# xuyuan/waymo_2d_tracking

Measured on AMD Instinct MI355X. Metric: end-to-end frames/sec (detect+SORT) on 1920x1280 Waymo frames, higher is better.
Workload: dtype f32; 1 GPU; Cascade R-CNN X152-32x8d-FPN dconv (random-init, fp32, batch 1) on synthetic 1920x1280x3 frames -> top-100 detections/frame -> SORT (max_age 2, min_hits 0, all boxes tracked; trackers resident for the whole segment); 5 cameras x 2 frames per step per GPU; 1x1 and dense 3x3 convolutions: f32 operands as exact 3 x bf16 splits, six cross terms on the bf16 matrix cores, f32 accumulate (csrc/det_gemm_s; stage=e2e, parallelism=sequence-shard x1

## Files before the change

### include/waymodet.h

```cpp
#ifndef WAYMODET_H
#define WAYMODET_H
#include <stddef.h>
#include <stdint.h>
#ifdef __cplusplus
extern "C" {
#endif

int wd_roi_pool_fpn_f32(const float* const* feats, const int32_t* heights, const int32_t* widths,
                        const float* scales, int n_levels, int channels, int batch,
                        const float* rois, int n_rois, int pooled, int min_level, int canonical_level,
                        float canonical_size, float* out, void* stream);

size_t wd_nms_workspace(int n);
int wd_select_kept(const uint8_t* keep_mask, const uint8_t* valid, const int64_t* order, int n, int cap, int64_t* out_idx,
                   int32_t* count, void* stream);
int wd_nms_sorted_f32(const float* boxes, const int32_t* idxs, int n, float iou_threshold,
                      uint8_t* keep_mask, int32_t* n_keep, void* workspace, size_t workspace_bytes, void* stream);

size_t wd_gemm_nt_workspace(int M, int N, int K);
int wd_gemm_nt_ws_f32(const float* A, const float* Bt, const float* bias, const float* residual, int relu, int M, int N, int K,
                      float* C, void* workspace, size_t workspace_bytes, void* stream);

int wd_gemm_lt_f32(const float* a, const float* w, const float* bias, const float* residual, float* out, int m, int n, int k,
                   int relu, void* workspace, size_t workspace_bytes, void* stream);
int wd_gemm_lt_plan_info(int m, int n, int k, int relu, int has_bias, int has_residual, float* best_us, int* candidates);
size_t wd_gemm_split_packed_bytes(int N, int K);
int wd_gemm_split_pack_weight(const float* w, int N, int K, void* packed, void* stream);
int wd_gemm_split_pack_weight_strided(const float* w, int N, int K, long stride_n, long stride_k, void* packed, void* stream);
typedef struct WdSplitPackDesc {
    const float* src;
    void* dst;
    long s_n, s_c, s_kh, s_kw;
    long first_block;
    int N, K, C, ksize, flip, reserved;
} WdSplitPackDesc;
int wd_gemm_split_pack_batch(const WdSplitPackDesc* descs_device, int count, long total_blocks, void* stream);
size_t wd_gemm_split_workspace(long M, int N, int K);
int wd_gemm_split_f32(const float* a, long lda, const void* packed_w, const float* bias, const float* residual, float* out, long ldc,
                      int M, int N, int K, int relu, void* workspace, size_t workspace_bytes, void* stream);
int wd_conv_split_f32(const float* x, int batch, int H, int W, int C, const void* packed_w, int ksize, int stride, int pad, const float* bias,
                      const float* residual, float* out, int N, int relu, void* workspace, size_t workspace_bytes, void* stream);
int wd_gemm_split_supported(const float* a, long lda, const float* bias, const float* residual, const float* out, long ldc, long M, int N, int K);
int wd_conv_split_position_major(int batch, int H, int W, int ksize, int stride, int pad);
typedef struct WdSplitIO {
    const float* a;
    long lda;
    const void* a_planes;
    const float* residual;
    const void* residual_planes;
    float* out;
    void* out_planes;
    long ldc;
} WdSplitIO;
size_t wd_split_planes_bytes(long M, int K);
int wd_split_planes_pack_f32(const float* a, long lda, long M, int K, void* planes, void* stream);
int wd_split_planes_unpack_f32(const void* planes, long M, int K, float* out, long ldo, void* stream);
int wd_gemm_split_io(const WdSplitIO* io, const void* packed_w, const float* bias, int M, int N, int K, int relu, void* workspace,
                     size_t workspace_bytes, void* stream);
int wd_nms_segmented_f32(const float* boxes, const int32_t* idxs, const int32_t* seg_offsets, int n_seg, float iou_threshold,
                         uint8_t* keep_mask, int32_t* n_keep, void* workspace, size_t workspace_bytes, void* stream);

size_t wd_rpn_topk_workspace(const int* n_per_level, int n_levels, int k);
int wd_rpn_topk_decode_f32(const float* const* logits, const float* const* deltas, const float* const* anchors,
                           const int* n_per_level, int n_levels, int k, float img_h, float img_w, float scale_clamp,
                           float* out_boxes, float* out_scores, int32_t* out_group, uint8_t* out_valid, void* workspace,
                           size_t workspace_bytes, void* stream);
int wd_sort_candidates_f32(const float* boxes, const float* scores, const int32_t* group, const uint8_t* valid,
                           const uint8_t* valid2 , int n, float* out_boxes, float* out_scores, int32_t* out_group, uint8_t* out_valid, int64_t* out_order,
                           void* stream);
int wd_box_candidates_f32(const float* boxes, const float* s0, const float* s1, const float* s2, const int32_t* n_valid, int rows,
                          int num_classes, float score_thresh, float img_h, float img_w, float* out_boxes, float* out_scores,
                          int32_t* out_group, uint8_t* out_valid, int64_t* out_order, void* stream);
int wd_gather_kept_f32(const uint8_t* keep, const uint8_t* valid, const float* boxes, const float* scores, const int64_t* order,
                       int n, int cap, int num_classes, float* out_boxes, float* out_scores, int64_t* out_class, int32_t* count,
                       void* stream);
int wd_detections_to_wire(const float* boxes, const float* scores, const int64_t* classes, const int32_t* count, int n, int in_w,
                          int in_h, int hflip, int out_w, int out_h, double* xywhs, int32_t* category, void* stream);

size_t wd_deform_packed_weight_floats(int c_in, int c_out, int groups);
int wd_deform_pack_weight(const float* weight_oihw, int c_in, int c_out, int groups, float* packed, void* stream);
const char* wd_deform_conv3x3_variant(int c_in, int groups, int stride, int pad, int has_offset);
const char* wd_deform_conv3x3_last_kernel(void);
int wd_deform_conv3x3_f32(const float* x, const float* offset, const float* mask, const float* packed_weight,
                          const float* scale, const float* bias, int relu,
                          int batch, int h, int w, int c_in, int c_out, int groups, int stride, int pad,
                          float* y, void* stream);
int wd_deform_conv3x3_hint_f32(const float* x, const float* offset, const float* mask, const float* packed_weight,
                               const float* scale, const float* bias, int relu, int batch, int h, int w, int c_in,
                               int c_out, int groups, int stride, int pad, int far_offsets, float* y, void* stream);
size_t wd_deform_table_bytes(int batch, int h, int w);
int wd_deform_offsets_table_f32(const float* partial, int ld, const float* bias, int batch, int h, int w, float* offsets,
                                void* table, void* stream);
int wd_deform_conv3x3_tab_f32(const float* x, const float* offset, const float* mask, const float* packed_weight,
                              const float* scale, const float* bias, int relu, int batch, int h, int w, int c_in,
                              int c_out, int groups, int stride, int pad, int far_offsets, const void* table, float* y,
                              void* stream);
// ... 57 lines not shown
```

### waymo_2d_tracking_amd/csrc/det_gemm_split.hip

```cpp
#include "common.h"
#include "../../include/waymodet.h"
#include <cstdlib>
#include <cstring>

namespace {

using bf16x8 = __attribute__((ext_vector_type(8))) __bf16;
using bf16x2 = __attribute__((ext_vector_type(2))) __bf16;
using f32x2 = __attribute__((ext_vector_type(2))) float;
using f32x16 = __attribute__((ext_vector_type(16))) float;
using u32x4 = __attribute__((ext_vector_type(4))) unsigned;

constexpr int BK = 64;
constexpr int BN = 256;
constexpr int NTHREADS = 512;
constexpr int CHUNK = 6144;

struct SplitArgs {
    const float* a;
    const unsigned char* ap;
    const uint4* w;
    const float* bias;
    const float* residual;
    const unsigned char* resp;
    float* out;
    unsigned char* outp;
    long lda, ldc;
    int M, N, K, relu;
    int tiles_m, tiles_n;
    int splitk;
    float* part;
    long long* stamps;
    int H, W, C, Ho, Wo, stride, pad, ksize;
};

__device__ __forceinline__ unsigned pk_bf16(float a, float b) {
    const f32x2 v = {a, b};
    return __builtin_bit_cast(unsigned, __builtin_convertvector(v, bf16x2));
}

__device__ __forceinline__ void split_pair(float x0, float x1, unsigned& h, unsigned& m, unsigned& l) {
    h = pk_bf16(x0, x1);
    const float r0 = x0 - __uint_as_float(h << 16), r1 = x1 - __uint_as_float(h & 0xffff0000u);
    m = pk_bf16(r0, r1);
    const float s0 = r0 - __uint_as_float(m << 16), s1 = r1 - __uint_as_float(m & 0xffff0000u);
    l = pk_bf16(s0, s1);
}

__device__ __forceinline__ float bf_lo(unsigned v) { return __uint_as_float(v << 16); }
__device__ __forceinline__ float bf_hi(unsigned v) { return __uint_as_float(v & 0xffff0000u); }

__device__ __forceinline__ size_t planes_offset(int row, int col, int ncols) {
    return ((size_t)(row >> 5) * (size_t)(ncols >> 5) + (size_t)(col >> 5)) * CHUNK +
           (size_t)((row & 31) * 64 + ((((col >> 3) & 3) ^ ((row >> 2) & 3)) << 4) + ((col >> 2) & 1) * 8);
}

constexpr int LDC = BN + 8;

template <int MT>
__device__ __forceinline__ void split_epilogue(const SplitArgs& p, unsigned char* smem, const f32x16 (&acc)[MT], int m0, int n0, int wave, int lane, int mlim,
                                               int row_mul = 1, int row_add = 0) {
    const int rr = lane & 31, rg = lane >> 5;
    float* ct = reinterpret_cast<float*>(smem);
    const int ncols = p.N - n0 < BN ? p.N - n0 : BN;
    constexpr int PASS = 3;
    auto stage = [&](int i0) {
        if (i0 > 0) __builtin_amdgcn_s_barrier();
#pragma unroll
        for (int i = i0; i < i0 + PASS && i < MT; ++i)
#pragma unroll
            for (int e = 0; e < 16; ++e)
                ct[((i - i0) * 32 + (e & 3) + 8 * (e >> 2) + 4 * rg) * LDC + 32 * wave + rr] = acc[i][e];
        __builtin_amdgcn_s_waitcnt(0xC07F);
        __builtin_amdgcn_s_barrier();
    };
    if (p.outp == nullptr) {
        const int c4 = 4 * lane;
        float4 bv = make_float4(0.f, 0.f, 0.f, 0.f);
        if (p.bias && c4 < ncols) bv = *reinterpret_cast<const float4*>(p.bias + n0 + c4);
        constexpr int RPW = 32 * PASS / 8;
#pragma unroll
        for (int i0 = 0; i0 < MT; i0 += PASS) {
            const int nrows = 32 * ((MT - i0) < PASS ? (MT - i0) : PASS);
            float4 rv[RPW];
            if (p.residual) {
// ... 64 lines not shown
        stage(i0);
#pragma unroll
        for (int j = 0; j < UPW; ++j) {
            const int u = wave + 8 * j;
            if (u < nunits && m0 + 32 * (i0 + u / (2 * ncb)) < mlim) {
                const int rbi = u / (2 * ncb), cb = (u >> 1) - rbi * ncb, h = u & 1;
                const int r = 16 * h + ur, row = m0 + 32 * (i0 + rbi) + r;
                const int c8 = 8 * ((lane & 3) ^ ((r >> 2) & 3)), col = n0 + 32 * cb + c8;
                const float* src = ct + (32 * rbi + r) * LDC + 32 * cb + c8;
                float4 v0 = *reinterpret_cast<const float4*>(src), v1 = *reinterpret_cast<const float4*>(src + 4);
                if (p.bias) {
                    const float4 b0 = *reinterpret_cast<const float4*>(p.bias + col), b1 = *reinterpret_cast<const float4*>(p.bias + col + 4);
                    v0.x += b0.x; v0.y += b0.y; v0.z += b0.z; v0.w += b0.w; v1.x += b1.x; v1.y += b1.y; v1.z += b1.z; v1.w += b1.w;
                }
                if (p.resp) {
                    const uint4 hh = rq[j][0], mm = rq[j][1], ll = rq[j][2];
                    v0.x += (bf_lo(hh.x) + bf_lo(mm.x)) + bf_lo(ll.x); v0.y += (bf_hi(hh.x) + bf_hi(mm.x)) + bf_hi(ll.x);
                    v0.z += (bf_lo(hh.y) + bf_lo(mm.y)) + bf_lo(ll.y); v0.w += (bf_hi(hh.y) + bf_hi(mm.y)) + bf_hi(ll.y);
                    v1.x += (bf_lo(hh.z) + bf_lo(mm.z)) + bf_lo(ll.z); v1.y += (bf_hi(hh.z) + bf_hi(mm.z)) + bf_hi(ll.z);
                    v1.z += (bf_lo(hh.w) + bf_lo(mm.w)) + bf_lo(ll.w); v1.w += (bf_hi(hh.w) + bf_hi(mm.w)) + bf_hi(ll.w);
                } else if (p.residual) {
                    const uint4 q0 = rq[j][0], q1 = rq[j][1];
                    v0.x += __uint_as_float(q0.x); v0.y += __uint_as_float(q0.y); v0.z += __uint_as_float(q0.z); v0.w += __uint_as_float(q0.w);
                    v1.x += __uint_as_float(q1.x); v1.y += __uint_as_float(q1.y); v1.z += __uint_as_float(q1.z); v1.w += __uint_as_float(q1.w);
                }
                if (p.relu) {
                    v0.x = fmaxf(v0.x, 0.f); v0.y = fmaxf(v0.y, 0.f); v0.z = fmaxf(v0.z, 0.f); v0.w = fmaxf(v0.w, 0.f);
                    v1.x = fmaxf(v1.x, 0.f); v1.y = fmaxf(v1.y, 0.f); v1.z = fmaxf(v1.z, 0.f); v1.w = fmaxf(v1.w, 0.f);
                }
                if (p.out && row < mlim) {
                    float4* d = reinterpret_cast<float4*>(p.out + (size_t)row * p.ldc + col);
                    d[0] = v0; d[1] = v1;
                }
                unsigned hv[4], mv[4], lv[4];
                split_pair(v0.x, v0.y, hv[0], mv[0], lv[0]); split_pair(v0.z, v0.w, hv[1], mv[1], lv[1]);
                split_pair(v1.x, v1.y, hv[2], mv[2], lv[2]); split_pair(v1.z, v1.w, hv[3], mv[3], lv[3]);
                unsigned char* q = p.outp + ((size_t)(row >> 5) * (size_t)(p.N >> 5) + (size_t)(col >> 5)) * CHUNK + h * 1024 + lane * 16;
                *reinterpret_cast<uint4*>(q) = make_uint4(hv[0], hv[1], hv[2], hv[3]);
                *reinterpret_cast<uint4*>(q + 2048) = make_uint4(mv[0], mv[1], mv[2], mv[3]);
                *reinterpret_cast<uint4*>(q + 4096) = make_uint4(lv[0], lv[1], lv[2], lv[3]);
            }
        }
    }
}

__device__ __forceinline__ int xcd_tile_id(int total) {
    const int x = blockIdx.x & 7, j = blockIdx.x >> 3;
    const int q = total >> 3, r = total & 7;
    if (j >= q + (x < r ? 1 : 0)) return -1;
    return (x < r ? x * (q + 1) : r * (q + 1) + (x - r) * q) + j;
}

template <int MT, int MODE>
__global__ __launch_bounds__(NTHREADS, 2) void gemm_split_kernel(const SplitArgs p) {
    extern __shared__ __attribute__((aligned(16))) unsigned char smem[];
    constexpr int BM = 32 * MT;
    constexpr int PLANE = BM * 64;
    constexpr int BUF = 3 * PLANE;
    const int tid = threadIdx.x, lane = tid & 63;
    const int wave = __builtin_amdgcn_readfirstlane(tid >> 6);
    constexpr bool CONV = MODE == 1 || MODE == 3;
    constexpr bool PM = MODE == 3;
    int id = PM ? (int)blockIdx.x : xcd_tile_id(p.tiles_m * p.tiles_n * p.splitk);
    if (id < 0 || (PM && id >= p.tiles_m * p.tiles_n)) return;
#ifdef WD_DEBUG
    long long t_start = 0, r_start = 0, t_main = 0, t_epi = 0;
    if (p.stamps) { t_start = __builtin_amdgcn_s_memtime(); r_start = __builtin_amdgcn_s_memrealtime(); }
    const int id_stamp = id;
#endif
    const int kz = PM ? 0 : id % p.splitk;
    if (!PM) id /= p.splitk;
    const int tm = id / p.tiles_n, tn = id - tm * p.tiles_n;
    int m0 = tm * BM;
    const int n0 = tn * BN;
    const int kc = CONV ? p.C / 32 : 1;
    int pm_y = 0, pm_x = 0, pm_nvt = 9;
    unsigned long long pm_taps = 0x876543210ull;
    if (PM) {
        const int nch = (p.M / (p.H * p.W) + BM - 1) / BM;
        const int wi = p.W - 2, hi = p.H - 2, ni = wi * hi, ne = 2 * wi + 2 * hi;
        int t = tm, c, q;
        if (t < ni * nch) { c = t / ni; q = t - c * ni; pm_y = 1 + q / wi; pm_x = 1 + q - (q / wi) * wi; }
        else if (t < (ni + ne) * nch) {
            t -= ni * nch; c = t / ne; q = t - c * ne;
            if (q < wi) { pm_y = 0; pm_x = 1 + q; }
            else if (q < 2 * wi) { pm_y = p.H - 1; pm_x = 1 + q - wi; }
            else if (q < 2 * wi + hi) { pm_x = 0; pm_y = 1 + q - 2 * wi; }
            else { pm_x = p.W - 1; pm_y = 1 + q - 2 * wi - hi; }
        } else { t -= (ni + ne) * nch; c = t >> 2; q = t & 3; pm_y = (q >> 1) ? p.H - 1 : 0; pm_x = (q & 1) ? p.W - 1 : 0; }
        m0 = c * BM;
        pm_taps = 0; pm_nvt = 0;
        for (int tp = 0; tp < 9; ++tp) {
            const int yy = pm_y + tp / 3 - 1, xx = pm_x + tp % 3 - 1;
            if (yy >= 0 && yy < p.H && xx >= 0 && xx < p.W) { pm_taps |= (unsigned long long)tp << (4 * pm_nvt); ++pm_nvt; }
        }
    }
    auto pm_tap = [&](int i) { return (int)((pm_taps >> (4 * i)) & 15ull); };
    const int nk_all = PM ? pm_nvt * kc : p.K / 32;
    const int per = (nk_all + p.splitk - 1) / p.splitk;
    const int k0 = kz * per;
    const int nk = (k0 + per <= nk_all) ? per : nk_all - k0;

    const int srow = tid >> 4, sk2 = tid & 15;
    unsigned aoff[MT];
    unsigned vmask[MT];
#pragma unroll
    for (int i = 0; i < MT; ++i) {
        int m = m0 + srow + 32 * i;
        if (PM) {
            const int maps = p.M / (p.H * p.W);
            m = m < maps ? m : maps - 1;
            aoff[i] = (unsigned)(((m * p.H + pm_y - 1) * p.W + pm_x - 1) * p.C + 2 * sk2);
            vmask[i] = 0x1ffu;
            continue;
        }
        m = m < p.M ? m : p.M - 1;
        if (MODE == 0) {
            aoff[i] = (unsigned)(m * p.lda) + 2u * sk2;
            vmask[i] = 1u;
        } else {
            const int hw = p.Ho * p.Wo;
            const int b = m / hw, rem = m - b * hw;
            const int yo = rem / p.Wo, xo = rem - yo * p.Wo;
            const int y0 = yo * p.stride - p.pad, x0 = xo * p.stride - p.pad;
            aoff[i] = (unsigned)(((b * p.H + y0) * p.W + x0) * p.C + 2 * sk2);
            unsigned vm = 0;
            for (int t = 0; t < p.ksize * p.ksize; ++t) {
                const int yy = y0 + t / p.ksize, xx = x0 + t % p.ksize;
                if (yy >= 0 && yy < p.H && xx >= 0 && xx < p.W) vm |= 1u << t;
            }
            vmask[i] = vm;
        }
    }
    float2 araw[MT];
    auto a_fetch = [&](int kt, int i) -> float2 {
        kt = k0 + (kt < nk ? kt : nk - 1);
        if (MODE == 0) {
            return *reinterpret_cast<const float2*>(p.a + (size_t)(aoff[i] + (unsigned)(kt * 32)));
        } else {
            const int ti = kt / kc, cb = kt - ti * kc;
            const int tap = PM ? pm_tap(ti) : ti;
            const int dy = tap / p.ksize, dx = tap - dy * p.ksize;
            const unsigned delta = (unsigned)((dy * p.W + dx) * p.C + cb * 32);
// ... 89 lines not shown
#ifdef WD_DEBUG
    if (p.stamps) t_main = __builtin_amdgcn_s_memtime();
#endif
    __builtin_amdgcn_s_waitcnt(0xC07F);
    __builtin_amdgcn_s_barrier();

    bf16x8 af[MT][3];
#define SB __builtin_amdgcn_sched_barrier(0)
#define MF(pa, pb, slot)                                                                                      \
    _Pragma("unroll") for (int i = 0; i < MT; ++i)                                                          \
        acc[i] = __builtin_amdgcn_mfma_f32_32x32x16_bf16(af[i][pa], wf[slot][pb], acc[i], 0, 0, 0);
#define RD(addr, pl)                                                                                          \
    _Pragma("unroll") for (int i = 0; i < MT; ++i)                                                          \
        af[i][pl] = *reinterpret_cast<const bf16x8*>(smem + (addr) + (pl) * PLANE + i * 2048);
#define SPLIT_ROW(i_)                                                                                         \
    if ((i_) < MT) { a_store_row(wr, (i_)); araw[(i_)] = aahead[(i_)]; aahead[(i_)] = CONV ? a_fetch_cur((i_)) : a_fetch(kt + 4, (i_)); }
    RD(rofs0, 2) RD(rofs0, 1) RD(rofs0, 0)
    SB;
    int cur = 0, nxt = BUF, wr = 2 * BUF;
    if (CONV) f_set(4);
    for (int kt = 0; kt < nk; ++kt) {
        const int a1 = cur + rofs1, a0n = nxt + rofs0;
        MF(2, 0, 0) RD(a1, 2) SB;
        MF(1, 1, 0) SPLIT_ROW(0) SB;
        MF(1, 0, 0) RD(a1, 1) SB;
        MF(0, 2, 0) SPLIT_ROW(1) SB;
        MF(0, 1, 0) SPLIT_ROW(2) SB;
        MF(0, 0, 0) RD(a1, 0) w_load(2 * kt + 2, 0); SB;
        MF(2, 0, 1) RD(a0n, 2) SB;
        MF(1, 1, 1) SPLIT_ROW(3) SB;
        MF(1, 0, 1) RD(a0n, 1) SB;
        MF(0, 2, 1) SPLIT_ROW(4) SB;
        MF(0, 1, 1) SPLIT_ROW(5) SB;
        MF(0, 0, 1) RD(a0n, 0) w_load(2 * kt + 3, 1); SB;
        __builtin_amdgcn_s_waitcnt(0xC07F | (MT << 8));
        __builtin_amdgcn_s_barrier();
        SB;
        const int t = cur; cur = nxt; nxt = wr; wr = t;
        if (CONV) f_advance(kt + 5);
    }
#undef SPLIT_ROW
#ifdef WD_DEBUG
    if (p.stamps) t_epi = __builtin_amdgcn_s_memtime();
#endif
    __builtin_amdgcn_s_waitcnt(0xC07F);
    __builtin_amdgcn_s_barrier();
    if (p.splitk > 1) {
        SplitArgs q = p;
        q.out = p.part + (size_t)kz * p.M * p.N;
        q.ldc = p.N;
        q.bias = nullptr; q.residual = nullptr; q.resp = nullptr; q.outp = nullptr; q.relu = 0;
        split_epilogue<MT>(q, smem, acc, m0, n0, wave, lane, p.M);
    } else if (PM) {
        split_epilogue<MT>(p, smem, acc, m0, n0, wave, lane, p.M / (p.H * p.W), p.H * p.W, pm_y * p.W + pm_x);
    } else {
        split_epilogue<MT>(p, smem, acc, m0, n0, wave, lane, p.M);
    }
#ifdef WD_DEBUG
    if (p.stamps && tid == 0) {
        long long* o = p.stamps + 8 * (long)blockIdx.x;
        o[0] = t_start; o[1] = t_main; o[2] = t_epi; o[3] = __builtin_amdgcn_s_memtime();
        o[4] = id_stamp; o[5] = __builtin_amdgcn_s_getreg(20  | (0 << 6) | (3 << 11));
        o[6] = r_start; o[7] = __builtin_amdgcn_s_memrealtime();
    }
#endif
}

#undef MF
#undef RD

template <int MT>
__global__ __launch_bounds__(NTHREADS, 2) void gemm_split_planes_kernel(const SplitArgs p) {
    extern __shared__ __attribute__((aligned(16))) unsigned char smem[];
    constexpr int BM = 32 * MT;
    constexpr int PLANE = BM * 64;
    constexpr int BUF = 3 * PLANE;
    constexpr int NPIECE = 6 * MT;
    constexpr int ND = (NPIECE + 7) / 8;
    const int tid = threadIdx.x, lane = tid & 63;
    const int wave = __builtin_amdgcn_readfirstlane(tid >> 6);
    int id = xcd_tile_id(p.tiles_m * p.tiles_n * p.splitk);
    if (id < 0) return;
#ifdef WD_DEBUG
    long long t_start = 0, r_start = 0, t_main = 0, t_epi = 0;
    if (p.stamps) { t_start = __builtin_amdgcn_s_memtime(); r_start = __builtin_amdgcn_s_memrealtime(); }
    const int id_stamp = id;
#endif
    const int kz = id % p.splitk;
    id /= p.splitk;
    const int tm = id / p.tiles_n, tn = id - tm * p.tiles_n;
    const int m0 = tm * BM, n0 = tn * BN;
    const int nk_all = p.K / 32;
    const int per = (nk_all + p.splitk - 1) / p.splitk;
    const int k0 = kz * per;
    const int nk = (k0 + per <= nk_all) ? per : nk_all - k0;

    const int nrb = (p.M + 31) >> 5;
    const size_t rb_stride = (size_t)nk_all * CHUNK;
    const unsigned char* dsrc[ND];
    unsigned ddst[ND];
#pragma unroll
    for (int j = 0; j < ND; ++j) {
        int c = wave + 8 * j;
        c = c < NPIECE ? c : NPIECE - 1;
        const int i = c / 6, pl = (c - 6 * i) >> 1, h = c & 1;
        int rb = tm * MT + i;
        rb = rb < nrb ? rb : nrb - 1;
        dsrc[j] = p.ap + (size_t)rb * rb_stride + (size_t)k0 * CHUNK + pl * 2048 + h * 1024;
        ddst[j] = (unsigned)(pl * PLANE + i * 2048 + h * 1024);
    }
    const unsigned lane16 = (unsigned)lane * 16u;
    auto dma16 = [&](const unsigned char* sbase, unsigned dst) {
        unsigned keep;
        asm volatile("s_mov_b32 %0, m0\n\ts_mov_b32 m0, %3\n\ts_nop 0\n\tglobal_load_lds_dwordx4 %1, %2\n\ts_mov_b32 m0, %0"
                     : "=&s"(keep) : "v"(lane16), "s"(sbase), "s"(dst) : "memory");
    };
    auto dma_piece = [&](int kt, unsigned bufoff, int j) {
        kt = kt < nk ? kt : nk - 1;
// ... 277 lines not shown
}

template <int MT, int MODE>
int launch(const SplitArgs& a, hipStream_t stream) {
    constexpr size_t lds_epi = 32u * (MT < 3 ? MT : 3) * LDC * 4u;
    constexpr size_t lds_ring = (MODE == 2 ? 4u : 3u) * 3u * 32u * MT * 64u;
    constexpr size_t lds = lds_ring > lds_epi ? lds_ring : lds_epi;
    const void* fn = MODE == 2 ? reinterpret_cast<const void*>(gemm_split_planes_kernel<MT>)
                               : reinterpret_cast<const void*>(gemm_split_kernel<MT, MODE == 2 ? 0 : MODE>);
    static wt::OncePerDevice attr;
    const int dev = wt::device_index();
    if (attr.needed(dev)) {
        WT_TRY(occupancy_guard(fn, MT));
        WT_HIP(hipFuncSetAttribute(fn, hipFuncAttributeMaxDynamicSharedMemorySize, (int)lds));
        attr.mark(dev);
    }
    const int total = a.tiles_m * a.tiles_n * a.splitk;
    const dim3 grid((unsigned)((total + 7) / 8 * 8));
    if constexpr (MODE == 2) hipLaunchKernelGGL((gemm_split_planes_kernel<MT>), grid, dim3(NTHREADS), lds, stream, a);
    else hipLaunchKernelGGL((gemm_split_kernel<MT, MODE>), grid, dim3(NTHREADS), lds, stream, a);
    WT_HIP(hipGetLastError());
    return WT_OK;
}

template <int MODE>
int dispatch(SplitArgs& a, void* workspace, size_t workspace_bytes, hipStream_t stream) {
#ifdef WD_DEBUG
    a.stamps = g_stamps;
#endif
    const bool can_split = workspace != nullptr && (a.N % 4) == 0;
    Plan pl = pick_plan(a.M, a.N, a.K, can_split);
    if (pl.splitk > 1 && workspace_bytes < (size_t)pl.splitk * a.M * a.N * sizeof(float)) pl = pick_plan(a.M, a.N, a.K, false);
    const int mt = pl.mt;
    a.splitk = pl.splitk;
    a.part = pl.splitk > 1 ? (float*)workspace : nullptr;
    a.tiles_m = (a.M + 32 * mt - 1) / (32 * mt);
    a.tiles_n = (a.N + BN - 1) / BN;
    int rc;
    switch (mt) {
        case 2: rc = launch<2, MODE>(a, stream); break;
        case 3: rc = launch<3, MODE>(a, stream); break;
        case 4: rc = launch<4, MODE>(a, stream); break;
        case 6: rc = launch<6, MODE>(a, stream); break;
        default: rc = launch<5, MODE>(a, stream); break;
    }
    if (rc != WT_OK || a.splitk == 1) return rc;
    const long mn4 = (long)a.M * a.N / 4;
    hipLaunchKernelGGL(gemm_split_reduce_kernel, dim3((unsigned)((mn4 + 255) / 256)), dim3(256), 0, stream, (const float4*)a.part, a.splitk, mn4, a.N / 4,
                       (const float4*)a.bias, a.residual, a.resp, a.ldc, a.relu, a.out, a.outp);
    WT_HIP(hipGetLastError());
    return WT_OK;
}

int dispatch_position_major(SplitArgs& a, hipStream_t stream) {
#ifdef WD_DEBUG
    a.stamps = g_stamps;
#endif
    const int maps = a.M / (a.H * a.W), kc = a.C / 32;
    const long tn = (a.N + BN - 1) / BN;
    const long ni = (long)(a.H - 2) * (a.W - 2), ne = 2l * (a.W - 2) + 2l * (a.H - 2);
    int best = 4;
    double best_t = 1e30;
    static const int forced_mt = experiment_knob("WD_SPLIT_MT");
    for (int mt = MT_MAX; mt >= MT_MIN; --mt) {
        if (forced_mt >= MT_MIN && forced_mt <= MT_MAX && mt != forced_mt) continue;
        const long nch = (maps + 32 * mt - 1) / (32 * mt);
        const double eff = (mt == 4 || mt == 5) ? 1.0 : 1.24;
        auto tile = [&](int taps) { return mt * taps * kc * 0.52 * eff + 2.0 + mt; };
        const double work = (double)nch * tn * (ni * tile(9) + ne * tile(6) + 4 * tile(4)) / 256.0;
        const double t = work > tile(9) ? work : tile(9);
        if (t < best_t * 0.97) { best_t = t; best = mt; }
    }
    a.splitk = 1; a.part = nullptr;
    a.tiles_m = a.H * a.W * ((maps + 32 * best - 1) / (32 * best));
    a.tiles_n = (int)tn;
    switch (best) {
        case 4: return launch<4, 3>(a, stream);
        case 6: return launch<6, 3>(a, stream);
        default: return launch<5, 3>(a, stream);
    }
}

bool misaligned(const void* p) { return (reinterpret_cast<uintptr_t>(p) & 15) != 0; }

}

extern "C" {

#ifdef WD_DEBUG
int wd_gemm_split_debug_stamps(long long* buf) {
    g_stamps = buf;
    return WT_OK;
}
#endif

size_t wd_gemm_split_packed_bytes(int N, int K) {
    if (N <= 0 || K <= 0 || (K % BK)) return 0;
    return (size_t)((N + 31) / 32) * 32 * (size_t)K * 6;
}

int wd_gemm_split_pack_weight_strided(const float* w, int N, int K, long stride_n, long stride_k, void* packed, void* stream_) {
    WT_TRY(wt::ensure_device());
    if (!w || !packed || N <= 0 || K <= 0 || (K % BK)) {
        wt::set_error("wd_gemm_split_pack_weight: K must be a positive multiple of %d (N=%d K=%d)", BK, N, K);
        return WT_ERR_INVALID;
    }
    const long total = (long)((N + 31) / 32) * 32 * (K / 8);
    hipLaunchKernelGGL(gemm_split_pack_kernel, dim3((unsigned)((total + 255) / 256)), dim3(256), 0, (hipStream_t)stream_, w, N, K, stride_n, stride_k,
                       (uint4*)packed, total);
    WT_HIP(hipGetLastError());
    return WT_OK;
}

int wd_gemm_split_pack_weight(const float* w, int N, int K, void* packed, void* stream_) {
    return wd_gemm_split_pack_weight_strided(w, N, K, (long)K, 1, packed, stream_);
}

int wd_gemm_split_pack_batch(const WdSplitPackDesc* descs_device, int count, long total_blocks, void* stream_) {
    WT_TRY(wt::ensure_device());
    if (count <= 0 || total_blocks <= 0) return WT_OK;
    if (!descs_device || total_blocks >= (1l << 31)) {
        wt::set_error("wd_gemm_split_pack_batch: NULL descriptor array or too many workgroups (%ld)", total_blocks);
        return WT_ERR_INVALID;
    }
    hipLaunchKernelGGL(gemm_split_pack_batch_kernel, dim3((unsigned)total_blocks), dim3(256), 0, (hipStream_t)stream_, descs_device, count);
    WT_HIP(hipGetLastError());
    return WT_OK;
}

size_t wd_gemm_split_workspace(long M, int N, int K) {
    if (M <= 0 || N <= 0 || K <= 0 || (K % BK) || (N % 32)) return 0;
    const Plan pl = pick_plan(M, N, K, true);
    return pl.splitk > 1 ? (size_t)pl.splitk * M * N * sizeof(float) : 0;
// ... 24 lines not shown
    return (size_t)((M + 31) / 32) * (size_t)(K / 32) * CHUNK;
}

int wd_split_planes_pack_f32(const float* a, long lda, long M, int K, void* planes, void* stream_) {
    WT_TRY(wt::ensure_device());
    if (!a || !planes || M <= 0 || M >= (1l << 31) || K <= 0 || (K % 32) || (lda & 3) || lda < K || misaligned(a) || misaligned(planes)) {
        wt::set_error("wd_split_planes_pack_f32: needs K %% 32 == 0 and 16-byte aligned rows (M=%ld K=%d lda=%ld)", M, K, lda);
        return WT_ERR_INVALID;
    }
    const long total = ((M + 31) / 32) * 32 * (K / 8);
    hipLaunchKernelGGL(split_planes_pack_kernel, dim3((unsigned)((total + 255) / 256)), dim3(256), 0, (hipStream_t)stream_, a, lda, (int)M, K,
                       (unsigned char*)planes, total);
    WT_HIP(hipGetLastError());
    return WT_OK;
}

int wd_split_planes_unpack_f32(const void* planes, long M, int K, float* out, long ldo, void* stream_) {
    WT_TRY(wt::ensure_device());
    if (!out || !planes || M <= 0 || M >= (1l << 31) || K <= 0 || (K % 32) || (ldo & 3) || ldo < K || misaligned(out) || misaligned(planes)) {
        wt::set_error("wd_split_planes_unpack_f32: needs K %% 32 == 0 and 16-byte aligned rows (M=%ld K=%d ldo=%ld)", M, K, ldo);
        return WT_ERR_INVALID;
    }
    const long total = M * (K / 8);
    hipLaunchKernelGGL(split_planes_unpack_kernel, dim3((unsigned)((total + 255) / 256)), dim3(256), 0, (hipStream_t)stream_, (const unsigned char*)planes,
                       (int)M, K, out, ldo, total);
    WT_HIP(hipGetLastError());
    return WT_OK;
}

int wd_gemm_split_io(const WdSplitIO* io, const void* packed_w, const float* bias, int M, int N, int K, int relu, void* workspace,
                     size_t workspace_bytes, void* stream_) {
    WT_TRY(wt::ensure_device());
    if (M <= 0 || N <= 0) return WT_OK;
    if (!io || !packed_w || misaligned(packed_w) || (!io->a && !io->a_planes) || (io->a && io->a_planes) || (!io->out && !io->out_planes) ||
        (io->residual && io->residual_planes) || K <= 0 || (K % BK) || (N % 32) || misaligned(io->a_planes) || misaligned(io->residual_planes) ||
        misaligned(io->out_planes) ||
        !wd_gemm_split_supported(io->a ? io->a : (const float*)packed_w, io->a ? io->lda : K, bias, io->residual, io->out, io->ldc ? io->ldc : N, M, N, K)) {
        wt::set_error("wd_gemm_split_io: exactly one of a / a_planes, at least one of out / out_planes, at most one residual form; K %% %d == 0, "
                      "N %% 32 == 0, 16-byte aligned pointers and rows (M=%d N=%d K=%d)", BK, M, N, K);
        return WT_ERR_INVALID;
    }
    SplitArgs s{};
    s.a = io->a; s.ap = (const unsigned char*)io->a_planes; s.w = (const uint4*)packed_w; s.bias = bias;
    s.residual = io->residual; s.resp = (const unsigned char*)io->residual_planes; s.out = io->out; s.outp = (unsigned char*)io->out_planes;
    s.lda = io->a ? io->lda : K; s.ldc = io->ldc ? io->ldc : N; s.M = M; s.N = N; s.K = K; s.relu = relu;
    return io->a ? dispatch<0>(s, workspace, workspace_bytes, (hipStream_t)stream_) : dispatch<2>(s, workspace, workspace_bytes, (hipStream_t)stream_);
}

int wd_conv_split_position_major(int batch, int H, int W, int ksize, int stride, int pad) {
    static const int no_pm = experiment_knob("WD_SPLIT_NO_POSMAJOR");
    return !no_pm && ksize == 3 && stride == 1 && pad == 1 && H >= 3 && W >= 3 && H * W <= 81 && batch >= 256;
}

int wd_conv_split_f32(const float* x, int batch, int H, int W, int C, const void* packed_w, int ksize, int stride, int pad, const float* bias,
                      const float* residual, float* out, int N, int relu, void* workspace, size_t workspace_bytes, void* stream_) {
    WT_TRY(wt::ensure_device());
    const int Ho = (H + 2 * pad - ksize) / stride + 1, Wo = (W + 2 * pad - ksize) / stride + 1;
    const long M = (long)batch * Ho * Wo;
    if (M <= 0 || N <= 0) return WT_OK;
    if (!x || !packed_w || !out || (ksize != 1 && ksize != 3) || stride < 1 || pad < 0 || C <= 0 || (C % BK) || (N % 32) || misaligned(x) ||
        misaligned(out) || misaligned(bias) || misaligned(residual) || (long)batch * H * W * C >= (1l << 31) || M >= (1l << 31)) {
        wt::set_error("wd_conv_split_f32: needs ksize 1 or 3, C %% %d == 0, N %% 32 == 0 and fewer than 2^31 input elements (C=%d N=%d k=%d)", BK, C, N, ksize);
        return WT_ERR_INVALID;
    }
    SplitArgs s{};
    s.a = x; s.w = (const uint4*)packed_w; s.bias = bias; s.residual = residual; s.out = out;
    s.lda = C; s.ldc = N; s.M = (int)M; s.N = N; s.K = ksize * ksize * C; s.relu = relu;
    s.H = H; s.W = W; s.C = C; s.Ho = Ho; s.Wo = Wo; s.stride = stride; s.pad = pad; s.ksize = ksize;
    if (wd_conv_split_position_major(batch, H, W, ksize, stride, pad)) return dispatch_position_major(s, (hipStream_t)stream_);
    return dispatch<1>(s, workspace, workspace_bytes, (hipStream_t)stream_);
}

}
```

Measured before the change: 43.40 frames/s.

## Schedule position-major conv tiles from a host-planned, cost-sorted tile table

Replaces the fixed, uniform-MT tiling of the position-major 3x3 conv with a host-side planner. The planner picks per-class (interior, edge, corner) row cuts that mix 4/5/6-block tiles, sorts the tiles by estimated cost and simulates the XCD/CU makespan to choose among cuts. The resulting tile table is uploaded once per device and read by the kernel, which dispatches the tile body specialised on row blocks. The aim is to reduce tail imbalance and padding waste in the RoI-head convolutions. The cost is a synchronous upload on first use, which fails under graph capture if the shape was not seen beforehand, plus a device table read per block.

```diff
diff --git a/include/waymodet.h b/include/waymodet.h
--- a/include/waymodet.h
+++ b/include/waymodet.h
@@ -42,6 +42,12 @@
                       const float* residual, float* out, int N, int relu, void* workspace, size_t workspace_bytes, void* stream);
 int wd_gemm_split_supported(const float* a, long lda, const float* bias, const float* residual, const float* out, long ldc, long M, int N, int K);
 int wd_conv_split_position_major(int batch, int H, int W, int ksize, int stride, int pad);
+int wd_conv_split_order_f32(const float* x, int batch, int H, int W, int C, const void* packed_w, int ksize, int stride, int pad, const float* bias,
+                            const float* residual, float* out, int N, int relu, int order, void* workspace, size_t workspace_bytes, void* stream);
+typedef struct WdSplitTile {
+    int first_map, rows, y, x, tile_n, taps, row_blocks, reserved;
+} WdSplitTile;
+int wd_gemm_split_tile_plan(int maps, int H, int W, int N, int C, WdSplitTile* tiles, int capacity, int* launch_row_blocks, double* makespan_us);
 typedef struct WdSplitIO {
     const float* a;
     long lda;
diff --git a/waymo_2d_tracking_amd/csrc/det_gemm_split.hip b/waymo_2d_tracking_amd/csrc/det_gemm_split.hip
--- a/waymo_2d_tracking_amd/csrc/det_gemm_split.hip
+++ b/waymo_2d_tracking_amd/csrc/det_gemm_split.hip
@@ -1,7 +1,13 @@
 #include "common.h"
 #include "../../include/waymodet.h"
+#include <algorithm>
 #include <cstdlib>
 #include <cstring>
+#include <map>
+#include <mutex>
+#include <tuple>
+#include <utility>
+#include <vector>
 
 namespace {
 
@@ -31,6 +37,7 @@
     int splitk;
     float* part;
     long long* stamps;
+    const WdSplitTile* tiles;
     int H, W, C, Ho, Wo, stride, pad, ksize;
 };
 
@@ -201,43 +208,23 @@
 }
 
 template <int MT, int MODE>
-__global__ __launch_bounds__(NTHREADS, 2) void gemm_split_kernel(const SplitArgs p) {
+__device__ __forceinline__ void split_tile(const SplitArgs& p, int m0, const int n0, const int kz, const int pm_y, const int pm_x,
+                                           const int mlim, const int wave, const int id_stamp) {
     extern __shared__ __attribute__((aligned(16))) unsigned char smem[];
     constexpr int BM = 32 * MT;
     constexpr int PLANE = BM * 64;
     constexpr int BUF = 3 * PLANE;
     const int tid = threadIdx.x, lane = tid & 63;
-    const int wave = __builtin_amdgcn_readfirstlane(tid >> 6);
     constexpr bool CONV = MODE == 1 || MODE == 3;
     constexpr bool PM = MODE == 3;
-    int id = PM ? (int)blockIdx.x : xcd_tile_id(p.tiles_m * p.tiles_n * p.splitk);
-    if (id < 0 || (PM && id >= p.tiles_m * p.tiles_n)) return;
 #ifdef WD_DEBUG
     long long t_start = 0, r_start = 0, t_main = 0, t_epi = 0;
     if (p.stamps) { t_start = __builtin_amdgcn_s_memtime(); r_start = __builtin_amdgcn_s_memrealtime(); }
-    const int id_stamp = id;
 #endif
-    const int kz = PM ? 0 : id % p.splitk;
-    if (!PM) id /= p.splitk;
-    const int tm = id / p.tiles_n, tn = id - tm * p.tiles_n;
-    int m0 = tm * BM;
-    const int n0 = tn * BN;
     const int kc = CONV ? p.C / 32 : 1;
-    int pm_y = 0, pm_x = 0, pm_nvt = 9;
+    int pm_nvt = 9;
     unsigned long long pm_taps = 0x876543210ull;
     if (PM) {
-        const int nch = (p.M / (p.H * p.W) + BM - 1) / BM;
-        const int wi = p.W - 2, hi = p.H - 2, ni = wi * hi, ne = 2 * wi + 2 * hi;
-        int t = tm, c, q;
-        if (t < ni * nch) { c = t / ni; q = t - c * ni; pm_y = 1 + q / wi; pm_x = 1 + q - (q / wi) * wi; }
-        else if (t < (ni + ne) * nch) {
-            t -= ni * nch; c = t / ne; q = t - c * ne;
-            if (q < wi) { pm_y = 0; pm_x = 1 + q; }
-            else if (q < 2 * wi) { pm_y = p.H - 1; pm_x = 1 + q - wi; }
-            else if (q < 2 * wi + hi) { pm_x = 0; pm_y = 1 + q - 2 * wi; }
-            else { pm_x = p.W - 1; pm_y = 1 + q - 2 * wi - hi; }
-        } else { t -= (ni + ne) * nch; c = t >> 2; q = t & 3; pm_y = (q >> 1) ? p.H - 1 : 0; pm_x = (q & 1) ? p.W - 1 : 0; }
-        m0 = c * BM;
         pm_taps = 0; pm_nvt = 0;
         for (int tp = 0; tp < 9; ++tp) {
             const int yy = pm_y + tp / 3 - 1, xx = pm_x + tp % 3 - 1;
@@ -433,9 +420,9 @@
         q.bias = nullptr; q.residual = nullptr; q.resp = nullptr; q.outp = nullptr; q.relu = 0;
         split_epilogue<MT>(q, smem, acc, m0, n0, wave, lane, p.M);
     } else if (PM) {
-        split_epilogue<MT>(p, smem, acc, m0, n0, wave, lane, p.M / (p.H * p.W), p.H * p.W, pm_y * p.W + pm_x);
+        split_epilogue<MT>(p, smem, acc, m0, n0, wave, lane, mlim, p.H * p.W, pm_y * p.W + pm_x);
     } else {
-        split_epilogue<MT>(p, smem, acc, m0, n0, wave, lane, p.M);
+        split_epilogue<MT>(p, smem, acc, m0, n0, wave, lane, mlim);
     }
 #ifdef WD_DEBUG
     if (p.stamps && tid == 0) {
@@ -445,6 +432,31 @@
         o[6] = r_start; o[7] = __builtin_amdgcn_s_memrealtime();
     }
 #endif
+}
+
+template <int MT, int MODE>
+__global__ __launch_bounds__(NTHREADS, 2) void gemm_split_kernel(const SplitArgs p) {
+    const int wave = __builtin_amdgcn_readfirstlane((int)threadIdx.x >> 6);
+    if constexpr (MODE == 3) {
+        const int id = (int)blockIdx.x;
+        if (id >= p.tiles_m) return;
+        const WdSplitTile* t = p.tiles + id;
+        const int m0 = __builtin_amdgcn_readfirstlane(t->first_map), rows = __builtin_amdgcn_readfirstlane(t->rows);
+        const int y = __builtin_amdgcn_readfirstlane(t->y), x = __builtin_amdgcn_readfirstlane(t->x);
+        const int n0 = __builtin_amdgcn_readfirstlane(t->tile_n) * BN;
+        const int nrb = (rows + 31) >> 5;
+        if (MT >= 6 && nrb >= 6) split_tile<(MT >= 6 ? 6 : MT), 3>(p, m0, n0, 0, y, x, m0 + rows, wave, id);
+        else if (MT >= 5 && nrb == 5) split_tile<(MT >= 5 ? 5 : MT), 3>(p, m0, n0, 0, y, x, m0 + rows, wave, id);
+        else split_tile<4, 3>(p, m0, n0, 0, y, x, m0 + rows, wave, id);
+    } else {
+        int id = xcd_tile_id(p.tiles_m * p.tiles_n * p.splitk);
+        if (id < 0) return;
+        const int id_stamp = id;
+        const int kz = id % p.splitk;
+        id /= p.splitk;
+        const int tm = id / p.tiles_n, tn = id - tm * p.tiles_n;
+        split_tile<MT, MODE>(p, tm * 32 * MT, tn * BN, kz, 0, 0, p.M, wave, id_stamp);
+    }
 }
 
 #undef MF
@@ -828,33 +840,210 @@
     return WT_OK;
 }
 
+double pm_tile_cost(int row_blocks, int taps, int kc) {
+    const int mt = row_blocks < MT_MIN ? MT_MIN : row_blocks;
+    const double eff = mt <= 5 ? 1.0 : 1.24;
+    return mt * taps * kc * 0.52 * eff + 2.0 + mt;
+}
+
+double pm_makespan(const std::vector<double>& cost) {
+    double freeat[256];
+    int heap_n[8];
+    for (int x = 0; x < 8; ++x) heap_n[x] = 0;
+    double end = 0.0;
+    for (size_t i = 0; i < cost.size(); ++i) {
+        const int x = (int)(i & 7);
+        double* h = freeat + 32 * x;
+        double start = 0.0;
+        if (heap_n[x] == 32) {
+            start = h[0];
+            h[0] = h[--heap_n[x]];
+            for (int k = 0;;) {
+                int c = 2 * k + 1;
+                if (c >= heap_n[x]) break;
+                if (c + 1 < heap_n[x] && h[c + 1] < h[c]) ++c;
+                if (h[k] <= h[c]) break;
+                const double t = h[k]; h[k] = h[c]; h[c] = t;
+                k = c;
+            }
+        }
+        const double fin = start + cost[i];
+        int k = heap_n[x]++;
+        h[k] = fin;
+        while (k > 0 && h[(k - 1) / 2] > h[k]) {
+            const double t = h[k]; h[k] = h[(k - 1) / 2]; h[(k - 1) / 2] = t;
+            k = (k - 1) / 2;
+        }
+        if (fin > end) end = fin;
+    }
+    return end;
+}
+
+std::vector<std::vector<int>> pm_cuts(int maps, int only_mt) {
+    std::vector<std::vector<int>> cuts;
+    auto add = [&](int n4, int n5, int n6) {
+        const int n = n4 + n5 + n6, cap = 128 * n4 + 160 * n5 + 192 * n6, least = n4 ? 128 : (n5 ? 160 : 192);
+        if (n == 0 || cap < maps || cap - least >= maps) return;
+        const int slack = cap - maps, each = slack / n, extra = slack % n;
+        std::vector<int> rows;
+        for (int j = 0; j < n; ++j) {
+            const int full = j < n6 ? 192 : (j < n6 + n5 ? 160 : 128);
+            const int r = full - each - (n - 1 - j < extra ? 1 : 0);
+            if (r <= 0) return;
+            rows.push_back(r);
+        }
+        if (std::find(cuts.begin(), cuts.end(), rows) == cuts.end()) cuts.push_back(rows);
+    };
+    const bool mixed = maps <= 3072 && !only_mt;
+    if (mixed) {
+        for (int n6 = 0; 192 * (n6 - 1) < maps; ++n6)
+            for (int n5 = 0; 192 * n6 + 160 * (n5 - 1) < maps; ++n5) {
+                const int rest = maps - 192 * n6 - 160 * n5;
+                add(rest > 0 ? (rest + 127) / 128 : 0, n5, n6);
+            }
+    } else {
+        for (int mt = MT_MAX; mt >= MT_MIN; --mt) {
+            if (only_mt && mt != only_mt) continue;
+            const int n = (maps + 32 * mt - 1) / (32 * mt);
+            add(mt == 4 ? n : 0, mt == 5 ? n : 0, mt == 6 ? n : 0);
+        }
+    }
+    return cuts;
+}
+
+struct PmPlan {
+    std::vector<WdSplitTile> tiles;
+    int mt = 5;
+    double makespan = 0.0;
+};
+
+void pm_build(int maps, int H, int W, int tn, int kc, const std::vector<int>* const cut[3], PmPlan* out, std::vector<double>* cost_out) {
+    std::vector<std::pair<int, int>> pos[3];
+    for (int y = 0; y < H; ++y)
+        for (int x = 0; x < W; ++x) {
+            const int ey = (y == 0 || y == H - 1), ex = (x == 0 || x == W - 1);
+            pos[ey + ex].push_back({y, x});
+        }
+    static const int taps_of[3] = {9, 6, 4};
+    struct Item { double cost; WdSplitTile t; };
+    std::vector<Item> items;
+    for (int cl = 0; cl < 3; ++cl) {
+        int m0 = 0;
+        for (int rows : *cut[cl]) {
+            const int rb = (rows + 31) / 32 < MT_MIN ? MT_MIN : (rows + 31) / 32;
+            const double c = pm_tile_cost(rb, taps_of[cl], kc);
+            for (const auto& yx : pos[cl])
+                for (int t = 0; t < tn; ++t) items.push_back({c, WdSplitTile{m0, rows, yx.first, yx.second, t, taps_of[cl], rb, 0}});
+            m0 += rows;
+        }
+    }
+    std::stable_sort(items.begin(), items.end(), [](const Item& a, const Item& b) { return a.cost > b.cost; });
+    cost_out->clear();
+    for (const Item& it : items) cost_out->push_back(it.cost);
+    if (out) {
+        out->tiles.clear();
+        out->mt = 5;
+        for (const Item& it : items) {
+            out->tiles.push_back(it.t);
+            if (it.t.row_blocks > out->mt) out->mt = it.t.row_blocks;
+        }
+    }
+}
+
+PmPlan plan_position_major(int maps, int H, int W, int N, int C) {
+    static const int forced = experiment_knob("WD_SPLIT_MT");
+    const int only_mt = (forced >= MT_MIN && forced <= MT_MAX) ? forced : 0;
+    const int tn = (N + BN - 1) / BN, kc = C / 32;
+    const std::vector<std::vector<int>> cuts = pm_cuts(maps, only_mt);
+    const int nc = (int)cuts.size();
+    std::vector<double> cost;
+    auto eval = [&](int a, int b, int c) {
+        const std::vector<int>* cut[3] = {&cuts[a], &cuts[b], &cuts[c]};
+        pm_build(maps, H, W, tn, kc, cut, nullptr, &cost);
+        double work = 0.0;
+        for (double c : cost) work += c;
+        return pm_makespan(cost) + 1e-7 * work;
+    };
+    int best[3] = {0, 0, 0};
+    double best_t = 1e30;
+    if ((long)nc * nc * nc <= 40000) {
+        for (int a = 0; a < nc; ++a)
+            for (int b = 0; b < nc; ++b)
+                for (int c = 0; c < nc; ++c) {
+                    const double t = eval(a, b, c);
+                    if (t < best_t) { best_t = t; best[0] = a; best[1] = b; best[2] = c; }
+                }
+    } else {
+        for (int a = 0; a < nc; ++a) {
+            const double t = eval(a, a, a);
+            if (t < best_t) { best_t = t; best[0] = best[1] = best[2] = a; }
+        }
+        for (int pass = 0; pass < 2; ++pass)
+            for (int cl = 0; cl < 3; ++cl)
+                for (int a = 0; a < nc; ++a) {
+                    int tr[3] = {best[0], best[1], best[2]};
+                    tr[cl] = a;
+                    const double t = eval(tr[0], tr[1], tr[2]);
+                    if (t < best_t) { best_t = t; best[cl] = a; }
+                }
+    }
+    PmPlan plan;
+    const std::vector<int>* cut[3] = {&cuts[best[0]], &cuts[best[1]], &cuts[best[2]]};
+    pm_build(maps, H, W, tn, kc, cut, &plan, &cost);
+    plan.makespan = pm_makespan(cost);
+    return plan;
+}
+
+struct PmKey {
+    int dev, maps, H, W, N, C;
+    bool operator<(const PmKey& o) const {
+        return std::tie(dev, maps, H, W, N, C) < std::tie(o.dev, o.maps, o.H, o.W, o.N, o.C);
+    }
+};
+std::mutex g_pm_mutex;
+std::map<PmKey, PmPlan> g_pm_plans;
+std::map<PmKey, const WdSplitTile*> g_pm_tables;
+
+const PmPlan& pm_plan_cached(int maps, int H, int W, int N, int C) {
+    const PmKey key{-1, maps, H, W, N, C};
+    auto it = g_pm_plans.find(key);
+    if (it == g_pm_plans.end()) it = g_pm_plans.emplace(key, plan_position_major(maps, H, W, N, C)).first;
+    return it->second;
+}
+
 int dispatch_position_major(SplitArgs& a, hipStream_t stream) {
 #ifdef WD_DEBUG
     a.stamps = g_stamps;
 #endif
-    const int maps = a.M / (a.H * a.W), kc = a.C / 32;
-    const long tn = (a.N + BN - 1) / BN;
-    const long ni = (long)(a.H - 2) * (a.W - 2), ne = 2l * (a.W - 2) + 2l * (a.H - 2);
-    int best = 4;
-    double best_t = 1e30;
-    static const int forced_mt = experiment_knob("WD_SPLIT_MT");
-    for (int mt = MT_MAX; mt >= MT_MIN; --mt) {
-        if (forced_mt >= MT_MIN && forced_mt <= MT_MAX && mt != forced_mt) continue;
-        const long nch = (maps + 32 * mt - 1) / (32 * mt);
-        const double eff = (mt == 4 || mt == 5) ? 1.0 : 1.24;
-        auto tile = [&](int taps) { return mt * taps * kc * 0.52 * eff + 2.0 + mt; };
-        const double work = (double)nch * tn * (ni * tile(9) + ne * tile(6) + 4 * tile(4)) / 256.0;
-        const double t = work > tile(9) ? work : tile(9);
-        if (t < best_t * 0.97) { best_t = t; best = mt; }
+    const int maps = a.M / (a.H * a.W);
+    const PmPlan* plan;
+    {
+        std::lock_guard<std::mutex> lock(g_pm_mutex);
+        plan = &pm_plan_cached(maps, a.H, a.W, a.N, a.C);
+        const PmKey key{wt::device_index(), maps, a.H, a.W, a.N, a.C};
+        auto it = g_pm_tables.find(key);
+        if (it == g_pm_tables.end()) {
+            hipStreamCaptureStatus cs = hipStreamCaptureStatusNone;
+            if (hipStreamIsCapturing(stream, &cs) != hipSuccess || cs != hipStreamCaptureStatusNone) {
+                (void)hipGetLastError();
+                wt::set_error("wd_conv_split_f32: position-major convolution %d maps x %d x %d, N=%d C=%d has no tile table on this device and the stream is "
+                              "being captured; run the shape once outside the capture (the table is allocated and uploaded by the first launch)",
+                              maps, a.H, a.W, a.N, a.C);
+                return WT_ERR_INVALID;
+            }
+            void* d = nullptr;
+            const size_t bytes = plan->tiles.size() * sizeof(WdSplitTile);
+            WT_HIP(hipMalloc(&d, bytes));
+            WT_HIP(hipMemcpyAsync(d, plan->tiles.data(), bytes, hipMemcpyHostToDevice, stream));
+            WT_HIP(hipStreamSynchronize(stream));
+            it = g_pm_tables.emplace(key, (const WdSplitTile*)d).first;
+        }
+        a.tiles = it->second;
     }
     a.splitk = 1; a.part = nullptr;
-    a.tiles_m = a.H * a.W * ((maps + 32 * best - 1) / (32 * best));
-    a.tiles_n = (int)tn;
-    switch (best) {
-        case 4: return launch<4, 3>(a, stream);
-        case 6: return launch<6, 3>(a, stream);
-        default: return launch<5, 3>(a, stream);
-    }
+    a.tiles_m = (int)plan->tiles.size();
+    a.tiles_n = 1;
+    return plan->mt >= 6 ? launch<6, 3>(a, stream) : launch<5, 3>(a, stream);
 }
 
 bool misaligned(const void* p) { return (reinterpret_cast<uintptr_t>(p) & 15) != 0; }
@@ -985,8 +1174,8 @@
     return !no_pm && ksize == 3 && stride == 1 && pad == 1 && H >= 3 && W >= 3 && H * W <= 81 && batch >= 256;
 }
 
-int wd_conv_split_f32(const float* x, int batch, int H, int W, int C, const void* packed_w, int ksize, int stride, int pad, const float* bias,
-                      const float* residual, float* out, int N, int relu, void* workspace, size_t workspace_bytes, void* stream_) {
+int wd_conv_split_order_f32(const float* x, int batch, int H, int W, int C, const void* packed_w, int ksize, int stride, int pad, const float* bias,
+                            const float* residual, float* out, int N, int relu, int order, void* workspace, size_t workspace_bytes, void* stream_) {
     WT_TRY(wt::ensure_device());
     const int Ho = (H + 2 * pad - ksize) / stride + 1, Wo = (W + 2 * pad - ksize) / stride + 1;
     const long M = (long)batch * Ho * Wo;
@@ -996,12 +1185,36 @@
         wt::set_error("wd_conv_split_f32: needs ksize 1 or 3, C %% %d == 0, N %% 32 == 0 and fewer than 2^31 input elements (C=%d N=%d k=%d)", BK, C, N, ksize);
         return WT_ERR_INVALID;
     }
+    if (order < 0 || order > 2 || (order == 2 && !(ksize == 3 && stride == 1 && pad == 1 && H >= 3 && W >= 3))) {
+        wt::set_error("wd_conv_split_order_f32: order is 0 (chosen by shape), 1 (row order) or 2 (position-major: 3x3 / stride 1 / pad 1, H and W >= 3)");
+        return WT_ERR_INVALID;
+    }
     SplitArgs s{};
     s.a = x; s.w = (const uint4*)packed_w; s.bias = bias; s.residual = residual; s.out = out;
     s.lda = C; s.ldc = N; s.M = (int)M; s.N = N; s.K = ksize * ksize * C; s.relu = relu;
     s.H = H; s.W = W; s.C = C; s.Ho = Ho; s.Wo = Wo; s.stride = stride; s.pad = pad; s.ksize = ksize;
-    if (wd_conv_split_position_major(batch, H, W, ksize, stride, pad)) return dispatch_position_major(s, (hipStream_t)stream_);
+    if (order == 2 || (order == 0 && wd_conv_split_position_major(batch, H, W, ksize, stride, pad))) return dispatch_position_major(s, (hipStream_t)stream_);
     return dispatch<1>(s, workspace, workspace_bytes, (hipStream_t)stream_);
 }
 
-}
+int wd_conv_split_f32(const float* x, int batch, int H, int W, int C, const void* packed_w, int ksize, int stride, int pad, const float* bias,
+                      const float* residual, float* out, int N, int relu, void* workspace, size_t workspace_bytes, void* stream_) {
+    return wd_conv_split_order_f32(x, batch, H, W, C, packed_w, ksize, stride, pad, bias, residual, out, N, relu, 0, workspace, workspace_bytes, stream_);
+}
+
+int wd_gemm_split_tile_plan(int maps, int H, int W, int N, int C, WdSplitTile* tiles, int capacity, int* launch_row_blocks, double* makespan_us) {
+    if (maps <= 0 || H < 3 || W < 3 || H * W > 81 || N <= 0 || (N % 32) || C <= 0 || (C % BK) || capacity < 0 || (capacity > 0 && !tiles)) {
+        wt::set_error("wd_gemm_split_tile_plan: needs maps > 0, 3 <= H, W and H * W <= 81, N %% 32 == 0, C %% %d == 0 (maps=%d H=%d W=%d N=%d C=%d)", BK, maps,
+                      H, W, N, C);
+        return -1;
+    }
+    std::lock_guard<std::mutex> lock(g_pm_mutex);
+    const PmPlan& plan = pm_plan_cached(maps, H, W, N, C);
+    const int n = (int)plan.tiles.size();
+    for (int i = 0; i < n && i < capacity; ++i) tiles[i] = plan.tiles[i];
+    if (launch_row_blocks) *launch_row_blocks = plan.mt;
+    if (makespan_us) *makespan_us = plan.makespan;
+    return n;
+}
+
+}
```

Result: no change. 43.43 frames/s (median of 2 runs) (+0.1%).
